# arkworks-rs/accumulation

Hardware: AMD Instinct MI355X
Metric: MSM throughput (point-scalar pairs/sec) at 2^20 Pallas (higher is better)
Workload: dtype u32; 1 GPU; 2^20-pair pallas MSM per GPU (north_star size; scalars uniform in [0, r), G_i = k_i*G), key resident + precomputed window multiples; pairs_per_gpu=1048576, curve=pallas, precomputed_key=True, parallelism=point-sharded x1, window_bits=20, pipeline=bucket-per-lane (k_prep_local_t + k_accum_bpl; skewed scalars re-run chunked), window_widths=9 x 20 + 4 x 19 bits = 256 (MsmGeom::n_narrow), msms_in_flight=3, full=False

## Files before the change

accumulation_amd/csrc/api_entry_ctx.inc:

```

const char* amsm_strerror(int s) {
  switch (s) {
    case AMSM_OK: return "ok";
    case AMSM_E_INVALID_ARG: return "invalid argument";
    case AMSM_E_OOM: return "out of (device) memory";
    case AMSM_E_HIP: return "HIP runtime error";
    case AMSM_E_UNSUPPORTED: return "unsupported size or configuration";
    case AMSM_E_NO_DEVICE: return "no usable gfx950 device (the host backend is never chosen implicitly: ask for AMSM_DEVICE_HOST)";
    case AMSM_E_SCALAR_RANGE: return "scalar out of range (not a canonical into_repr value)";
    case AMSM_E_RCCL: return "RCCL collective failed";
    case AMSM_E_INVALID_POINT: return "invalid point (non-canonical, off the curve or outside the prime-order subgroup)";
    default: return "unknown error";
  }
}

int amsm_device_count(void) {
  int n = 0;
  if (hipGetDeviceCount(&n) != hipSuccess) {
    (void)hipGetLastError();
    return 0;
  }
  return n;
}

// ... 61 lines not shown
  {
    hipDeviceProp_t prop;
    if (hipGetDeviceProperties(&prop, device_id) == hipSuccess && prop.multiProcessorCount > 0) {
      c->cu_count = prop.multiProcessorCount;
      int per_cu = with_curve(curve, [](auto cv) { return accum_l0_blocks_per_cu<typename decltype(cv)::Fq>(); });
      c->wave_slots = prop.multiProcessorCount * std::max(1, per_cu) * 4;
    }
  }
  c->pool_cap_bytes = pool_cap_from_env(c->pool_cap_bytes);
  c->gate.limit = mem_limit_from_env();
  if (const char* e = getenv("AMSM_BPL")) c->bpl = atoi(e) != 0;
  if (const char* e = getenv("AMSM_BPL_PLAIN")) c->bpl_plain = atoi(e) != 0;
  if (const char* e = getenv("AMSM_TOP_SETS")) {
    const int t = atoi(e);
    c->top_sets = (t == 2 || t == 4 || t == 8) ? t : 0;
  }
  if (const char* e = getenv("AMSM_BPL_PROBE")) c->bpl_probe = atoi(e) != 0;
  if (const char* e = getenv("AMSM_BPS")) c->bps = std::max(0, std::min(2, atoi(e)));
  if (const char* e = getenv("AMSM_BPS_BATCH")) c->bps_batch = std::max(0, std::min((int)msel::BPS_BATCH, atoi(e)));
  if (const char* e = getenv("AMSM_SPLIT_LOG2")) c->split_log2 = std::max(0, std::min(28, atoi(e)));
  if (const char* e = getenv("AMSM_DIRECT_SUM_MAX_LOG2")) c->direct_max_log2 = std::max(0, std::min(16, atoi(e)));
  if (const char* e = getenv("AMSM_TWO_VALUED")) c->two_valued = atoi(e) != 0;
  if (const char* e = getenv("AMSM_SHARE_BUCKETS")) c->share_buckets = atoi(e) != 0;
  if (const char* e = getenv("AMSM_HOST_HALVES")) c->host_halves = atoi(e) != 0;
  if (const char* e = getenv("AMSM_SUBGROUP_LADDER")) c->subgroup_ladder = atoi(e) == 2 ? 2 : 1;
  if (const char* e = getenv("AMSM_VEC_SAMPLE_FORM")) c->vec_sample_form = std::max(0, std::min(2, atoi(e)));
  *out = c;
  return AMSM_OK;
}

// ... 282 lines not shown
```

accumulation_amd/csrc/api_pipeline.inc:

```

#define HIP_TRY(expr)                                                                                  \
  do {                                                                                                 \
    hipError_t _e = (expr);                                                                            \
    if (_e != hipSuccess) {                                                                            \
      fprintf(stderr, "[amsm] HIP error %s (%d) at %s:%d: %s\n", hipGetErrorName(_e), (int)_e, __FILE__, \
              __LINE__, #expr);                                                                        \
      return _e == hipErrorOutOfMemory ? AMSM_E_OOM : AMSM_E_HIP;                                      \
    }                                                                                                  \
  } while (0)

#define TRY(expr)            \
  do {                       \
    int _s = (expr);         \
    if (_s != AMSM_OK) return _s; \
  } while (0)

int ensure(DevBuf& b, size_t bytes) {
  if (b.bytes >= bytes && b.p) return AMSM_OK;
  if (b.p) HIP_TRY(gate_free(b.p));
  b.p = nullptr;
  b.bytes = 0;
  size_t want = bytes + bytes / 8 + 256;
  TRY(gate_alloc(b.owner, GATE_DEVICE, want, false, &b.p));
  b.bytes = want;
// ... 473 lines not shown
  u32* d_heavy_count = d_err + 1;
  u32* vals_a = (u32*)sl->vals_a.p;
  u32* vals_b = (u32*)sl->vals_b.p;

  auto prep = [&]() -> int {
    if (!short_prep) HIP_TRY(hipMemsetAsync(sl->misc.p, 0, 64, st));
    stage_mark(ctx, sl, ST_DIGITS, st);
    if (g.bpl) {
      PrepBplBuffers pb;
      pb.d_small = d_err + 16;
      pb.part = vals_a;
      pb.ents_t = vals_b;
      pb.grp = sl->bpl_grp.p;
      pb.order = (u32*)sl->bpl_order.p;
      pb.err = d_err;
      const int rc = g.bpl == 2 ? launch_prep_bps<Fr>(st, (const u32*)d_scalars, scalars_mont, g, g.bps_log2_l, pb)
                                : launch_prep_bpl<Fr>(st, (const u32*)d_scalars, scalars_mont, g, pb);
      if (rc != 0) return AMSM_E_HIP;
      stage_mark(ctx, sl, ST_SORT, st);
      stage_mark(ctx, sl, ST_BOUNDS, st);
      if (g.bpl != 2) ctx->n_bpl++;
      else if (!job.counted) ctx->n_bps++;
      if (g.bpl == 1u && g.top_split) ctx->n_top_sets[(g.top_split + 1u) / 4u]++;
    } else if (short_prep) {
      PrepBuffers pb;
      pb.d_small = d_err + 16;
      pb.part = vals_a;
      pb.vals_sorted = vals_b;
      pb.start = (u32*)sl->start.p;
      pb.items = (u32*)sl->items.p;
// ... 1117 lines not shown
```

accumulation_amd/csrc/api_types.h:

```cpp
#pragma once
struct amsm_ctx;
namespace {

enum Stage { ST_DIGITS = 0, ST_SORT, ST_BOUNDS, ST_ACCUM_L0, ST_ACCUM_L12, ST_REDUCE, ST_COUNT };
const char* kStageNames[ST_COUNT] = {"prep_chain", "prep_sort_rocprim", "prep_bounds_rocprim", "accum_l0", "accum_l1_l2",
                                     "bucket_reduce_fold"};

struct DevBuf {
  void* p = nullptr;
  size_t bytes = 0;
  amsm_ctx* owner = nullptr;
  void release();
};

struct MemGate {
  size_t held = 0, peak = 0;
  size_t limit = 0;
  size_t pinned = 0;
  unsigned long long requests = 0, refused_limit = 0, refused_hook = 0, failed_driver = 0;
  long fail_after = -1;
};

}

// ... 147 lines not shown
struct amsm_ctx {
  int curve = 0;
  int device = 0;
  bool host_only = false;
  hipStream_t stream = nullptr;
  hipStream_t s_prep = nullptr;
  hipStream_t s_tail = nullptr;
  bool own_stream = false;
  int window_override = 0;
  int cu_count = 256;
  unsigned vec_grid_max = 0;
  int wave_slots = 4096;
  bool bpl = true;
  bool bpl_plain = true;
  int top_sets = 0;
  int bps = 2;
  int split_log2 = 21;
  unsigned long long n_bps = 0, n_bps_fallbacks = 0;
  int bps_batch = msel::BPS_BATCH;
  unsigned long long n_bps_units = 0, n_bps_batched = 0, n_bps_unit_reruns = 0;
  unsigned long long n_direct = 0;
  int direct_max_log2 = 15;
  unsigned direct_rr = 0;
  bool host_halves = true;
  bool bpl_probe = true;
  unsigned long long n_top_sets[3] = {0, 0, 0};
  unsigned long long n_bpl = 0, n_bpl_fallbacks = 0;
  bool share_buckets = true;
  DevBuf shared_buckets[2];
  hipEvent_t shared_free[2] = {};
// ... 120 lines not shown
```

accumulation_amd/csrc/kern_fr.hip:

```cpp
#include "launch.h"
#include "vec_kernels.h"
#include "prep_kernels.h"

#include <algorithm>
#include <cmath>
#include <atomic>
#include <cstdlib>
#include <cstring>

namespace amsm {

static inline u32 cdiv_(u32 a, u32 b) { return (a + b - 1) / b; }
void launch_bounds(hipStream_t st, const void* keys_sorted, bool keys16, u32* vals_sorted, MsmGeom g, u32* start,
                   u32* items) {
  if (keys16)
    hipLaunchKernelGGL((k_bounds<uint16_t>), dim3(cdiv_(g.B, 256)), dim3(256), 0, st, (const uint16_t*)keys_sorted,
                       vals_sorted, g, start, items);
  else
    hipLaunchKernelGGL((k_bounds<u32>), dim3(cdiv_(g.B, 256)), dim3(256), 0, st, (const u32*)keys_sorted, vals_sorted,
                       g, start, items);
}

constexpr u32 PREP_MAX_P = 4096;
static PrepGeom prep_geom(const MsmGeom& g) {
// ... 2 lines not shown
  while (((g.B + (1u << pg.SH) - 1u) >> pg.SH) > 512u && pg.SH < 10u) pg.SH++;
  while (((g.B + (1u << pg.SH) - 1u) >> pg.SH) > PREP_MAX_P) pg.SH++;
  pg.P = (g.B + (1u << pg.SH) - 1u) >> pg.SH;
  pg.SPB = g.S <= 16u ? 512u : 256u;
  unsigned long long max_idx = (unsigned long long)g.base_off + g.n - 1ull +
                               (g.precomp ? (unsigned long long)(g.W - 1u) * g.table_stride : 0ull);
  if (g.idx_rel_bits) max_idx = ((unsigned long long)(g.W - 1u) << g.idx_rel_bits) | ((1ull << g.idx_rel_bits) - 1ull);
  pg.IB = 1;
  while ((max_idx >> pg.IB) != 0ull) pg.IB++;
  while (pg.IB + pg.SH > 31u && pg.SH > 0u && ((g.B + (1u << (pg.SH - 1)) - 1u) >> (pg.SH - 1)) <= PREP_MAX_P) pg.SH--;
  pg.P = (g.B + (1u << pg.SH) - 1u) >> pg.SH;
  const u32 budget_words = 37888u, fixed_words = 2u * (1u << pg.SH) + 1024u;
  pg.CAP = budget_words > fixed_words + 4096u ? budget_words - fixed_words : 0u;
  pg.HEAVY = std::max<u32>(4u * (g.E / pg.P + 1u), 1u << 17);
  pg.FIX = 0;
  return pg;
}
static size_t prep_heavy_words(const MsmGeom& g) { return (size_t)g.B + 4096 + 64; }
size_t prep_small_words(const MsmGeom& g) { return 4 * (PREP_MAX_P + 1) + 1 + 3 * prep_heavy_words(g) + PREP_MAX_HEAVY; }
static size_t prep_local_lds(const PrepGeom& pg) { return (2 * (size_t)(1u << pg.SH) + 1024 + pg.CAP) * sizeof(u32); }
constexpr size_t PREP_LDS_LIMIT = 160 * 1024;
static std::atomic<unsigned long long> prep_local_attr_devices{0};
static void prep_local_attr() {
  int dev = 0;
  if (hipGetDevice(&dev) != hipSuccess || dev < 0 || dev >= 64) dev = 63;
  const unsigned long long bit = 1ull << dev;
  if (dev != 63 && (prep_local_attr_devices.load(std::memory_order_acquire) & bit)) return;
  (void)hipFuncSetAttribute((const void*)k_prep_local, hipFuncAttributeMaxDynamicSharedMemorySize, 152 * 1024);
  prep_local_attr_devices.fetch_or(bit, std::memory_order_release);
}
// ... 1 lines not shown
  const size_t cap = (size_t)pg.SPB * g.S;
  return (3 * (size_t)pg.P + cap) * sizeof(u32) + cap * sizeof(uint16_t);
}
bool prep_supported(const MsmGeom& g) {
  if (g.n == 0 || g.S > 32u) return false;
  PrepGeom pg = prep_geom(g);
  return pg.SH <= 12u && pg.IB + pg.SH <= 31u && prep_scatter_lds(g, pg) <= PREP_LDS_LIMIT &&
         prep_local_lds(pg) <= PREP_LDS_LIMIT && (pg.P + 256) * sizeof(u32) <= 64 * 1024;
}

constexpr u32 BPL_LOCAL_FIXED_WORDS = 3u * BPL_NB + 2u * BPL_BINS + 2u * BPL_GROUPS + 2u;
constexpr u32 BPL_LOCAL_BUDGET_WORDS = 40960u;
static_assert(BPL_LOCAL_BUDGET_WORDS - BPL_LOCAL_FIXED_WORDS <= BPL_LOCAL_SLOTS * BPL_NB,
              "k_prep_local_t keeps a partition of CAP entries in BPL_LOCAL_SLOTS registers per lane");
static_assert(BPL_LOCAL_BUDGET_WORDS - BPL_LOCAL_FIXED_WORDS == msel::BPL_STAGE_CAP, "msm_select.h plans for k_prep_local_t's stage");
static PrepGeom prep_bpl_geom(const MsmGeom& g) {
  PrepGeom pg;
  pg.SH = 10;
  pg.P = g.B >> pg.SH;
  pg.SPB = g.S <= 16u ? 512u : 256u;
  unsigned long long max_idx = (unsigned long long)g.base_off + g.n - 1ull +
                               (g.precomp ? (unsigned long long)(g.W - 1u) * g.table_stride : 0ull);
  if (g.idx_rel_bits) max_idx = ((unsigned long long)(g.W - 1u) << g.idx_rel_bits) | ((1ull << g.idx_rel_bits) - 1ull);
  pg.IB = 1;
  while ((max_idx >> pg.IB) != 0ull) pg.IB++;
  pg.CAP = BPL_LOCAL_BUDGET_WORDS - BPL_LOCAL_FIXED_WORDS;
  pg.HEAVY = 0xffffffffu;
  const unsigned long long per = std::max<unsigned long long>(((unsigned long long)g.E + pg.P - 1) / std::max(1u, pg.P), g.part_max);
  pg.FIX = (u32)std::min<unsigned long long>(pg.CAP, (per + per / 4ull + 2048ull + 15ull) & ~15ull);
  return pg;
}
size_t prep_bpl_part_entries(const MsmGeom& g) {
  PrepGeom pg = prep_bpl_geom(g);
  return std::max<size_t>(g.E, pg.FIX ? (size_t)pg.P * pg.FIX : 0);
}
static size_t prep_bpl_local_lds(const PrepGeom& pg) { return (size_t)(BPL_LOCAL_FIXED_WORDS + pg.CAP) * sizeof(u32); }
static size_t prep_bpl_scatter_lds(const MsmGeom& g, const PrepGeom& pg) {
  const size_t cap = (size_t)pg.SPB * g.S;
  return (3 * (size_t)pg.P + 2 * cap) * sizeof(u32) + cap * sizeof(uint16_t);
}
u32 prep_bpl_partitions(const MsmGeom& g) { return g.B >> 10; }
u32 prep_bpl_groups_per_partition() { return BPL_GROUPS; }
u32 prep_bpl_stride(const MsmGeom& g) {
  const u32 P = std::max(1u, prep_bpl_partitions(g));
// ... 6 lines not shown
  PrepGeom pg = prep_bpl_geom(g);
  if (pg.IB > 30u) return false;
  if (!msel::bpl_stage_fits(g.E, pg.P, g.part_max, pg.CAP)) return false;
  return prep_bpl_scatter_lds(g, pg) <= PREP_LDS_LIMIT && prep_bpl_local_lds(pg) <= PREP_LDS_LIMIT &&
         (unsigned long long)pg.P * prep_bpl_stride(g) < (1ull << 31);
}
static std::atomic<unsigned long long> prep_bpl_attr_devices{0};
template <class KS>
static void prep_bpl_attr(KS scatter_kernel) {
  int dev = 0;
  if (hipGetDevice(&dev) != hipSuccess || dev < 0 || dev >= 64) dev = 63;
  const unsigned long long bit = 1ull << dev;
  (void)hipFuncSetAttribute((const void*)scatter_kernel, hipFuncAttributeMaxDynamicSharedMemorySize, (int)PREP_LDS_LIMIT);
  if (dev != 63 && (prep_bpl_attr_devices.load(std::memory_order_acquire) & bit)) return;
  static_assert((BPL_LOCAL_BUDGET_WORDS) * sizeof(u32) <= PREP_LDS_LIMIT, "k_prep_local_t's LDS must fit a workgroup");
  (void)hipFuncSetAttribute((const void*)k_prep_local_t, hipFuncAttributeMaxDynamicSharedMemorySize, (int)PREP_LDS_LIMIT);
  prep_bpl_attr_devices.fetch_or(bit, std::memory_order_release);
}

constexpr u32 bps_local_fixed_words(u32 nbp) { return 4u * nbp + 1024u + BPL_BINS + 2u * BPS_GROUPS + 2u; }
constexpr u32 BPS_LOCAL_BUDGET_WORDS = 37888u;
static PrepGeom prep_bps_geom(const MsmGeom& g, u32 log2_l) {
  PrepGeom pg;
  pg.SH = 10u - log2_l;
  pg.P = g.B >> pg.SH;
  pg.SPB = g.S <= 16u ? 512u : 256u;
  unsigned long long max_idx = (unsigned long long)g.base_off + g.n - 1ull +
                               (g.precomp ? (unsigned long long)(g.W - 1u) * g.table_stride : 0ull);
  if (g.idx_rel_bits) max_idx = ((unsigned long long)(g.W - 1u) << g.idx_rel_bits) | ((1ull << g.idx_rel_bits) - 1ull);
  pg.IB = 1;
  while ((max_idx >> pg.IB) != 0ull) pg.IB++;
  pg.CAP = BPS_LOCAL_BUDGET_WORDS - bps_local_fixed_words(1u << pg.SH);
  pg.HEAVY = 0xffffffffu;
  const unsigned long long per = ((unsigned long long)g.E + pg.P - 1) / std::max(1u, pg.P);
  pg.FIX = (u32)std::min<unsigned long long>(pg.CAP, (per + per / 2ull + 1024ull + 15ull) & ~15ull);
  return pg;
}
size_t prep_bps_part_entries(const MsmGeom& g, u32 log2_l) {
  PrepGeom pg = prep_bps_geom(g, log2_l);
  return std::max<size_t>(g.E, pg.FIX ? (size_t)pg.P * pg.FIX : 0);
}
static size_t prep_bps_local_lds(const PrepGeom& pg) {
  return (size_t)(bps_local_fixed_words(1u << pg.SH) + pg.CAP) * sizeof(u32);
}
u32 prep_bps_partitions(const MsmGeom& g, u32 log2_l) { return g.B >> (10u - log2_l); }
u32 prep_bps_stride(const MsmGeom& g, u32 log2_l) {
  const u32 P = std::max(1u, prep_bps_partitions(g, log2_l));
  const unsigned long long per = ((unsigned long long)g.E + P - 1) / P;
  return (u32)((per + per / 2ull + 4096ull + 1023ull) & ~1023ull);
}
// ... 174 lines not shown
    if (hipMemsetAsync(b.small, 0, (size_t)nv * b.small_stride * sizeof(u32), st) != hipSuccess) return -1;          \
    prep_bps_attr();                                                                                                 \
    const size_t lds_scatter = prep_scatter_lds(g, pg);                                                              \
    if (lds_scatter > 64 * 1024)                                                                                     \
      (void)hipFuncSetAttribute((const void*)k_prep_scatter_batch<FR, 16, 1>, hipFuncAttributeMaxDynamicSharedMemorySize, \
                                (int)PREP_LDS_LIMIT);                                                                \
    hipLaunchKernelGGL((k_prep_scatter_batch<FR, 16, 1>), dim3(cdiv_(g.n, pg.SPB), nv), dim3(512), lds_scatter, st, sc, mont, g,   \
                       pg, part_start0, part_cursor0, b.small_stride, b.part, b.part_stride, b.small);               \
    hipLaunchKernelGGL(k_prep_local_s_batch, dim3(pg.P, nv), dim3(1024), prep_bps_local_lds(pg), st, part_cursor0,   \
                       b.small_stride, b.part, b.part_stride, g, pg, stride, log2_l, b.ents_t, b.ents_stride,        \
                       (BplGroup*)b.grp, b.grp_stride, b.order, b.order_stride, b.small);                            \
    return 0;                                                                                                        \
  }                                                                                                                  \
  template <>                                                                                                        \
  int launch_prep_bpl<FR>(hipStream_t st, const u32* scalars, int mont, MsmGeom g, const PrepBplBuffers& b) {        \
    PrepGeom pg = prep_bpl_geom(g);                                                                                  \
    u32* part_total = b.d_small;                                                                                     \
    u32* part_start = b.d_small + (PREP_MAX_P + 1);                                                                  \
    u32* part_cursor = b.d_small + 2 * (PREP_MAX_P + 1);                                                             \
    PrepHeavy hv;                                                                                                    \
    hv.n = b.d_small + 4 * (PREP_MAX_P + 1);                                                                         \
    hv.cnt = hv.n + 1;                                                                                               \
    hv.ids = hv.cnt + 64;                                  \
    hv.cur = hv.end = hv.ids;                                                                                        \
    {                  \
      size_t zero_bytes = (16 + 4 * (PREP_MAX_P + 1) + 1) * sizeof(u32);                                             \
      zero_bytes = (zero_bytes + 255) & ~(size_t)255;                                                                \
      if (b.err != b.d_small - 16) return -1;                                                                        \
      if (hipMemsetAsync(b.err, 0, zero_bytes, st) != hipSuccess) return -1;                                         \
    }                                                                                                                \
    if (g.S <= 16u) prep_bpl_attr(k_prep_scatter<FR, 16, 1, true>);                                                  \
    else prep_bpl_attr(k_prep_scatter<FR, 32, 1, true>);                                                             \
    if (!pg.FIX) {                                                                                                   \
      PrepGeom ph = pg;                                                                                              \
      ph.SPB = 1024;                                                                                                 \
      hipLaunchKernelGGL((k_prep_hist<FR>), dim3(cdiv_(g.n, 1024)), dim3(1024), pg.P * sizeof(u32), st, scalars,      \
                         mont, g, ph, part_total, b.err);                                                            \
      hipLaunchKernelGGL(k_prep_scan, dim3(1), dim3(1024), 0, st, part_total, part_start, pg.P, pg.HEAVY, hv);       \
    }                                                                                                                \
    if (g.S <= 16u)                                                                                                  \
      hipLaunchKernelGGL((k_prep_scatter<FR, 16, 1, true>), dim3(cdiv_(g.n, pg.SPB)), dim3(512),                     \
                         prep_bpl_scatter_lds(g, pg), st, scalars, mont, g, pg, part_start, part_cursor, b.part, b.err); \
    else                                             \
      hipLaunchKernelGGL((k_prep_scatter<FR, 32, 1, true>), dim3(cdiv_(g.n, pg.SPB)), dim3(256),                     \
                         prep_bpl_scatter_lds(g, pg), st, scalars, mont, g, pg, part_start, part_cursor, b.part, b.err); \
    hipLaunchKernelGGL(k_prep_local_t, dim3(pg.P), dim3(1024), prep_bpl_local_lds(pg), st,                           \
                       pg.FIX ? part_cursor : part_start, (const u64*)b.part, g, pg, prep_bpl_stride(g), b.ents_t,   \
                       (BplGroup*)b.grp, b.order, b.err);                                                            \
    return 0;                                                                                                        \
  }                                                                                                                  \
  template <>                                                                                                        \
  void launch_digits<FR>(hipStream_t st, const u32* scalars, int mont, MsmGeom g, void* keys, bool keys16, u32* vals, \
                         u32* err) {                                                                                 \
    if (keys16)                                                                                                      \
      hipLaunchKernelGGL((k_digits<FR, uint16_t>), dim3(cdiv_(g.n, 256)), dim3(256), 0, st, scalars, mont, g,         \
                         (uint16_t*)keys, vals, err);                                                                \
    else                                                                                                             \
      hipLaunchKernelGGL((k_digits<FR, u32>), dim3(cdiv_(g.n, 256)), dim3(256), 0, st, scalars, mont, g, (u32*)keys,  \
                         vals, err);                                                                                 \
  }                                                                                                                  \
  template <>                                                                                                        \
  void launch_skew_probe<FR>(hipStream_t st, const u32* scalars, int mont, u32 n, DigitWalk walk, u32* d_flag,       \
                             const u32* d_tv_words) {                                                               \
// ... 125 lines not shown
```

accumulation_amd/csrc/launch.h:

```cpp
#pragma once
#include <hip/hip_runtime.h>

#include <algorithm>

#include "blind.h"
#include "msm_select.h"
#include "msm_types.h"

namespace amsm {

template <class Fq>
void launch_accum_l0(hipStream_t st, const u32* table, const u32* vals_sorted, const u32* start,
                     const u32* item_off, MsmGeom g, u32* partials);
template <class Fq>
void launch_accum_bpl(hipStream_t st, const u32* table, const u32* ents_t, const void* grp, const u32* order, u32 n_groups,
                      u32 groups_per_part, const u32* flags, u32* buckets, u32 wg_per_cu = 0, bool accumulate = false);
template <class Fq>
int accum_l0_blocks_per_cu();
template <class Fq>
void launch_accum_l1(hipStream_t st, u32 lanes_per_bucket, const u32* partials, const u32* items, const u32* item_off, MsmGeom g,
                     u32* buckets, u32* heavy_count, u32* heavy_list);
template <class Fq>
void launch_accum_l2(hipStream_t st, const u32* partials, const u32* items, const u32* item_off,
                     const u32* heavy_count, const u32* heavy_list, u32* scratch, u32* buckets);
// ... 63 lines not shown
  u32* part;
  u32* vals_sorted;
  u32* start;
  u32* items;
  u32* item_off;
  u32* err;
};
bool prep_supported(const MsmGeom& g);
struct PrepBplBuffers {
  u32* d_small;
  u32* part;
  u32* ents_t;
  void* grp;
  u32* order;
  u32* err;
};
bool prep_bpl_supported(const MsmGeom& g);
u32 prep_bpl_stride(const MsmGeom& g);
u32 prep_bpl_partitions(const MsmGeom& g);
size_t prep_bpl_part_entries(const MsmGeom& g);
size_t prep_bps_part_entries(const MsmGeom& g, u32 log2_l);
u32 prep_bpl_groups_per_partition();
template <class Fr>
int launch_prep_bpl(hipStream_t st, const u32* scalars, int mont, MsmGeom g, const PrepBplBuffers& b);
int prep_bps_choose(const MsmGeom& g);
u32 prep_bps_partitions(const MsmGeom& g, u32 log2_l);
u32 prep_bps_stride(const MsmGeom& g, u32 log2_l);
template <class Fr>
int launch_prep_bps(hipStream_t st, const u32* scalars, int mont, MsmGeom g, u32 log2_l, const PrepBplBuffers& b);
template <class Fq>
// ... 81 lines not shown
```

accumulation_amd/csrc/msm_select.h:

```cpp
#pragma once
#include <math.h>
#include <stddef.h>

#include <initializer_list>

namespace amsm {
namespace msel {

enum Pipeline { DIRECT_SUM = 0, BUCKET_SPLIT = 1, BUCKET_PER_LANE = 2, CHUNKED = 3 };
inline const char* pipeline_name(int p) {
  return p == DIRECT_SUM ? "direct_sum" : (p == BUCKET_SPLIT ? "bucket_split" : (p == BUCKET_PER_LANE ? "bucket_per_lane" : "chunked"));
}

inline int ilog2_ceil(size_t n) {
  int l = 0;
  while (((size_t)1 << l) < n) l++;
  return l;
}
constexpr size_t P2(int k) { return (size_t)1 << k; }

constexpr int BPL_WINDOW = 20;
constexpr int DIRECT_MAX_LOG2 = 15;
struct KeyWindowRow {
  int lg_lo, lg_hi;
// ... 211 lines not shown
  const unsigned long long per_top = ((unsigned long long)n * 1024ull + reach - 1) / reach;
  const unsigned long long top = (2ull * per_top + T - 1) / T;
  const unsigned long long pm = per_win > top ? per_win : top;
  return groups > 1u ? (pm + 1ull) / 2ull : pm;
}
inline unsigned plain_top_sets(size_t n, unsigned nb, unsigned long long reach, unsigned W, unsigned groups, unsigned cap = BPL_STAGE_CAP,
                               unsigned max_sets = 8) {
  if (n == 0 || nb < 1024u || reach == 0 || W == 0) return 0;
  for (unsigned T = 2; T <= max_sets && T <= 8u; T *= 2u) {
    const unsigned long long P = ((unsigned long long)groups * (W + T) * nb) >> 10;
    if (bpl_stage_fits((unsigned long long)n * W, P, plain_part_max(n, nb, reach, T, groups), cap)) return T;
  }
  return 0;
}
inline unsigned plain_top_sets_cap(int top_sets) { return top_sets == 2 ? 2u : 8u; }

enum class Place {
  LONE,
  BATCH_LAST,
  BATCH_INNER,
};
inline Place place_of(size_t i, size_t count) { return count == 1 ? Place::LONE : (i + 1 == count ? Place::BATCH_LAST : Place::BATCH_INNER); }
enum TailForm {
  RED2 = 0,
  FUSED_QUAD = 1,
  ONE_LANE = 2
};
inline const char* tail_form_name(int f) { return f == RED2 ? "red2" : (f == FUSED_QUAD ? "fused_quad" : "one_lane"); }
constexpr int TAIL_QUAD_HIDDEN_LOG2 = 17;
constexpr unsigned RED2_COLS = 1024, RED2_MIN_NB = 1u << 18;
// ... 65 lines not shown
```

accumulation_amd/csrc/prep_kernels.h:

```cpp
#pragma once
#include "fp.h"
#include "msm_select.h"
#include "msm_types.h"
#include "vec_kernels.h"

namespace amsm {

struct PrepGeom {
  u32 SH;
  u32 P;
  u32 SPB;
  u32 IB;
  u32 CAP;
  u32 HEAVY;
  u32 FIX;
};

constexpr u32 PREP_HEAVY_SLICES = 64, PREP_HEAVY_GRID = 1024, PREP_MAX_HEAVY = 4096;
struct PrepHeavy {
  u32* n;
  u32* ids;
  u32* cnt;
  u32* cur;
  u32* end;
};

constexpr u32 PREP_ENTRY_LAST = 0x40000000u;

AMSM_DEV u32 lds_count(u32* ctr, u32 idx) {
  const u64 active = __ballot(1);
// ... 91 lines not shown
    u32 v = in[k];
    out[k] = run;
    run += v;
  }
  if (with_total && t == T - 1) out[n] = lds[T - 1];
}

__global__ void __launch_bounds__(1024)
    k_prep_scan(const u32* __restrict__ part_total, u32* __restrict__ part_start, u32 P, u32 heavy_min, PrepHeavy hv) {
  __shared__ u32 lds[1024];
  block_exclusive_scan(part_total, part_start, P, true, lds);
  for (u32 p = threadIdx.x; p < P; p += blockDim.x)
    if (part_total[p] > heavy_min) hv.ids[atomicAdd(hv.n, 1u)] = p;
}

template <class Fr, int MAXW, int SPT, bool WIDE>
AMSM_DEV void prep_scatter_body(const u32* scalars, int mont, MsmGeom g, PrepGeom pg, const u32* part_start, u32* part_cursor, u32* part,
                                u32* err) {
  extern __shared__ u32 prep_lds[];
  const u32 cap = pg.SPB * g.S;
  u32* cnt = prep_lds;
  u32* loff = prep_lds + pg.P;
  u32* gbase = prep_lds + 2 * pg.P;
  u32* staged = prep_lds + 3 * pg.P;
  uint16_t* staged_p = reinterpret_cast<uint16_t*>(staged + (WIDE ? 2u : 1u) * cap);
  const u32 t = threadIdx.x, T = blockDim.x;
  for (u32 p = t; p < pg.P; p += T) cnt[p] = 0;
  __syncthreads();
  u32 rk[SPT][MAXW / 2];
  Fe<Fr> sreg[SPT];
// ... 2 lines not shown
#pragma unroll
    for (int k = 0; k < MAXW / 2; k++) rk[r][k] = 0;
    u32 i = blockIdx.x * pg.SPB + r * T + t;
    if (i < g.n) {
      sreg[r] = fe_load<Fr>(scalars + (size_t)i * 8);
      if (g.skip_ones) fe_drop_stored_one<Fr>(sreg[r], mont);
      if (mont) sreg[r] = fe_from_mont<Fr>(sreg[r]);
      const u32 bad = scalar_entries_unrolled_reg<Fr, MAXW>(sreg[r], g, i, [&](int w, u32 key, u32) {
        u32 rank = atomicAdd(&cnt[key >> pg.SH], 1u);
        rk[r][w >> 1] |= rank << ((w & 1) * 16);
      });
      if (pg.FIX && bad && err) atomicOr(err, 1u);
    }
  }
  __syncthreads();
  constexpr u32 RSV_MAX = 4;
  u32 rsv[RSV_MAX], rsv_base[RSV_MAX];
  u32 per = (pg.P + T - 1) / T;
  u32 lo = min(t * per, pg.P), hi = min(lo + per, pg.P);
  {
    u32* sl = reinterpret_cast<u32*>(staged);
    u32 sum = 0;
    for (u32 p = lo; p < hi; p++) sum += cnt[p];
    sl[t] = sum;
    __syncthreads();
    for (u32 d = 1; d < T; d <<= 1) {
      u32 v = t >= d ? sl[t - d] : 0u;
      __syncthreads();
      sl[t] += v;
      __syncthreads();
    }
    u32 run = sl[t] - sum;
#pragma unroll
    for (u32 q = 0; q < RSV_MAX; q++) {
      u32 p = lo + q;
      rsv[q] = 0;
      rsv_base[q] = 0;
      if (p < hi) {
        u32 v = cnt[p];
        loff[p] = run;
        if (v) {
          rsv_base[q] = pg.FIX ? p * pg.FIX : part_start[p];
          rsv[q] = atomicAdd(&part_cursor[p], v);
        }
        run += v;
      }
    }
    for (u32 p = lo + RSV_MAX; p < hi; p++) {
      u32 v = cnt[p];
      loff[p] = run;
      gbase[p] = v ? (pg.FIX ? p * pg.FIX : part_start[p]) + atomicAdd(&part_cursor[p], v) : 0u;
      run += v;
    }
  }
  __syncthreads();
  const u32 low = (1u << pg.SH) - 1u;
#pragma unroll
  for (int r = 0; r < SPT; r++) {
    u32 i = blockIdx.x * pg.SPB + r * T + t;
    if (i < g.n)
      scalar_entries_unrolled_reg<Fr, MAXW>(sreg[r], g, i, [&](int w, u32 key, u32 val) {
        u32 p = key >> pg.SH;
        u32 rank = (rk[r][w >> 1] >> ((w & 1) * 16)) & 0xffffu;
        u32 slot = loff[p] + rank;
        if (WIDE) reinterpret_cast<u64*>(staged)[slot] = ((u64)(key & low) << 32) | val;
        else staged[slot] = (val & 0x80000000u) | ((key & low) << pg.IB) | (val & 0x7fffffffu);
        staged_p[slot] = (uint16_t)p;
      });
  }
#pragma unroll
  for (u32 q = 0; q < RSV_MAX; q++)
    if (lo + q < hi) gbase[lo + q] = rsv_base[q] + rsv[q];
  __syncthreads();
  u32 total = loff[pg.P - 1] + cnt[pg.P - 1];
  for (u32 j = t; j < total; j += T) {
    u32 p = staged_p[j];
    const u32 dst = gbase[p] + (j - loff[p]);
    if (pg.FIX && dst - p * pg.FIX >= pg.FIX) continue;
    if (WIDE) reinterpret_cast<u64*>(part)[dst] = reinterpret_cast<const u64*>(staged)[j];
    else part[dst] = staged[j];
  }
}
template <class Fr, int MAXW, int SPT, bool WIDE = false>
__global__ void __launch_bounds__(512)
    k_prep_scatter(const u32* __restrict__ scalars, int mont, MsmGeom g, PrepGeom pg, const u32* __restrict__ part_start,
                   u32* __restrict__ part_cursor, u32* __restrict__ part, u32* __restrict__ err = nullptr) {
  prep_scatter_body<Fr, MAXW, SPT, WIDE>(scalars, mont, g, pg, part_start, part_cursor, part, err);
}
constexpr int PREP_BPS_BATCH = msel::BPS_BATCH;
struct BpsBatchScalars {
  const u32* scalars[PREP_BPS_BATCH];
};
template <class Fr, int MAXW, int SPT>
// ... 236 lines not shown
  u32 m;
};
AMSM_DEV void bpl_slot(u32 s, u32& pos, u32& half) {
  if (s < BPL_SPLIT) {
    pos = s >> 1;
    half = 1u + (s & 1u);
  } else if (s >= BPL_NB) {
    pos = BPL_SPLIT / 2u + ((s - BPL_NB) >> 1);
    half = 1u + (s & 1u);
  } else {
    pos = s;
    half = 0u;
  }
}

AMSM_DEV u32 block_scan_inclusive(u32 v, u32* wt) {
  const u32 lane = __lane_id(), w = threadIdx.x >> 6;
#pragma unroll
  for (u32 d = 1; d < 64u; d <<= 1) {
    const u32 o = __shfl_up(v, d);
    if (lane >= d) v += o;
  }
  if (lane == 63u) wt[w] = v;
  __syncthreads();
  u32 before = 0;
#pragma unroll
  for (u32 i = 0; i < 15u; i++) before += i < w ? wt[i] : 0u;
  return v + before;
}

constexpr u32 BPL_LOCAL_SLOTS = 37, BPL_SLOT_BLOCK = 8;
template <class F>
AMSM_DEV void bpl_slot_blocks(u32 n, F&& f) {
#pragma unroll
  for (u32 b = 0; b < BPL_LOCAL_SLOTS; b += BPL_SLOT_BLOCK)
    if (b * BPL_NB < n) f(b);
}

__global__ void __launch_bounds__(1024)
    k_prep_local_t(const u32* __restrict__ part_start, const u64* __restrict__ part, MsmGeom g, PrepGeom pg, u32 stride,
                   u32* __restrict__ ents_t, BplGroup* __restrict__ grp, u32* __restrict__ order, u32* __restrict__ err) {
  extern __shared__ u32 prep_lds[];
  constexpr u32 NB = BPL_NB, NG = BPL_GROUPS, T = BPL_NB, SLOTS = BPL_LOCAL_SLOTS, BLK = BPL_SLOT_BLOCK;
  u32* cnt = prep_lds;
  u32* cur = cnt + NB;
  u32* wt = cur + NB;
  u32* bins = wt + NB;
  u32* first = bins + BPL_BINS;
  u32* gm = first + BPL_BINS;
  u32* stage = gm + 2u * NG + 1u;
  const u32 p = blockIdx.x, t = threadIdx.x;
  const u32 ps = pg.FIX ? p * pg.FIX : part_start[p];
  const u32 n_p = pg.FIX ? part_start[p] : part_start[p + 1] - ps;
  const u32 pe = ps + (pg.FIX ? min(n_p, pg.FIX) : n_p);
  const u32 low = NB - 1u, idx_mask = (1u << pg.IB) - 1u, b0 = p << pg.SH;
  const bool fits = n_p <= pg.CAP && (!pg.FIX || n_p <= pg.FIX);
  const u32 n = fits ? min(pe - ps, SLOTS * T) : 0u;
  u64 e[SLOTS];
#pragma unroll
  for (u32 i = 0; i < SLOTS; i++) e[i] = 0;
  bpl_slot_blocks(n, [&](u32 b) {
#pragma unroll
    for (u32 i = b; i < b + BLK && i < SLOTS; i++) e[i] = part[ps + min(i * T + t, n - 1u)];
  });
  cnt[t] = 0;
  if (t < BPL_BINS) bins[t] = 0;
  if (t < NG) gm[t] = 0;
  __syncthreads();
  bpl_slot_blocks(n, [&](u32 b) {
#pragma unroll
    for (u32 i = b; i < b + BLK && i < SLOTS; i++)
      if (i * T + t < n) atomicAdd(&cnt[(u32)(e[i] >> 32) & low], 1u);
  });
  __syncthreads();
  const u32 c_t = cnt[t];
  const u32 first_t = block_scan_inclusive(c_t, wt) - c_t;
  cur[t] = first_t;
  const u32 bin = min(c_t, BPL_BINS - 1u);
  const u32 rank = atomicAdd(&bins[bin], 1u);
  __syncthreads();
  bpl_slot_blocks(n, [&](u32 b) {
    u32 pos[BLK];
#pragma unroll
    for (u32 i = b; i < b + BLK && i < SLOTS; i++) {
      pos[i - b] = 0;
      if (i * T + t < n) pos[i - b] = atomicAdd(&cur[(u32)(e[i] >> 32) & low], 1u);
    }
#pragma unroll
    for (u32 i = b; i < b + BLK && i < SLOTS; i++) {
      const u32 lo = (u32)e[i];
      if (i * T + t < n) stage[pos[i - b]] = (lo & 0x80000000u) | entry_abs_index(g, lo & idx_mask);
    }
  });
  const u32 in_class = t < BPL_BINS ? bins[BPL_BINS - 1u - t] : 0u;
  const u32 larger = block_scan_inclusive(in_class, wt + 16) - in_class;
  if (t < BPL_BINS) first[BPL_BINS - 1u - t] = larger;
  __syncthreads();
  const u32 my_pos = first[bin] + rank;
  cnt[my_pos] = c_t;
  cur[my_pos] = first_t;
  {
    const u32 h0 = (c_t + 1u) >> 1;
    if (my_pos < BPL_SPLIT / 2u) atomicMax(&gm[0], h0);
    else if (my_pos < BPL_SPLIT) atomicMax(&gm[NG - 1u], h0);
    else atomicMax(&gm[my_pos / BPL_GROUP], c_t);
  }
// ... 7 lines not shown
  const bool ok = fits && total <= stride;
  if (!ok && t == 0) atomicOr(err + 1, 1u);
  if (t < NG) {
    BplGroup h;
    h.base = p * stride + my_gb;
    h.m = ok ? gm[t] : 0u;
    grp[p * NG + t] = h;
  }
  {
    u32* o = order + (size_t)p * BPL_LANES;
    if (my_pos < BPL_SPLIT / 2u) o[2u * my_pos] = o[2u * my_pos + 1u] = b0 + t;
    else if (my_pos < BPL_SPLIT) o[BPL_NB + 2u * (my_pos - BPL_SPLIT / 2u)] = o[BPL_NB + 2u * (my_pos - BPL_SPLIT / 2u) + 1u] = b0 + t;
    else o[my_pos] = b0 + t;
  }
  if (!ok) return;
  const u32 w = t >> 6, l = t & 63u;
  auto slot_of = [&](u32 q, u32& sz, u32& src) {
    u32 pos, half;
    bpl_slot(q * BPL_GROUP + l, pos, half);
    const u32 c = cnt[pos], h0 = (c + 1u) >> 1;
    sz = half == 0u ? c : (half == 1u ? h0 : c - h0);
    src = cur[pos] + (half == 2u ? h0 : 0u);
  };
  u32* out = ents_t + (size_t)p * stride + l;
  u32 row0 = 0, sz, src, m = gm[0];
  slot_of(0, sz, src);
  for (u32 q = 0; q < NG; q++) {
    u32 sz_n = 0, src_n = 0, m_n = 0;
    if (q + 1u < NG) {
      m_n = gm[q + 1u];
      slot_of(q + 1u, sz_n, src_n);
// ... 125 lines not shown
```

Baseline: 1.009 billion pairs/s.

## Shard per-partition scatter cursors across blocks to cut global atomic contention

The scatter kernel now splits each fixed-size partition into several sub-regions, each with its own cursor, chosen by block index, so scattering blocks contend on separate global atomic counters. The local transpose kernel gains a sharded variant that rebuilds a per-slot validity mask from the shard counts, because entries are no longer contiguous. The shard count is picked from a statistical margin check on expected fill, and the scatter block scan is replaced with a wave-shuffle scan. The costs are gaps inside partitions, extra validity bookkeeping, and a higher overflow risk for unevenly distributed digits.

```diff
diff --git a/accumulation_amd/csrc/api_entry_ctx.inc b/accumulation_amd/csrc/api_entry_ctx.inc
--- a/accumulation_amd/csrc/api_entry_ctx.inc
+++ b/accumulation_amd/csrc/api_entry_ctx.inc
@@ -99,6 +99,10 @@
   if (const char* e = getenv("AMSM_TOP_SETS")) {
     const int t = atoi(e);
     c->top_sets = (t == 2 || t == 4 || t == 8) ? t : 0;
+  }
+  if (const char* e = getenv("AMSM_PREP_SHARDS")) {
+    const int s = atoi(e);
+    c->prep_shards = (s == 1 || s == 2 || s == 4 || s == 8 || s == 16) ? s : 0;
   }
   if (const char* e = getenv("AMSM_BPL_PROBE")) c->bpl_probe = atoi(e) != 0;
   if (const char* e = getenv("AMSM_BPS")) c->bps = std::max(0, std::min(2, atoi(e)));
diff --git a/accumulation_amd/csrc/api_pipeline.inc b/accumulation_amd/csrc/api_pipeline.inc
--- a/accumulation_amd/csrc/api_pipeline.inc
+++ b/accumulation_amd/csrc/api_pipeline.inc
@@ -511,6 +511,7 @@
       pb.grp = sl->bpl_grp.p;
       pb.order = (u32*)sl->bpl_order.p;
       pb.err = d_err;
+      pb.shards = ctx->prep_shards ? ctx->prep_shards : (one ? 0 : 1);
       const int rc = g.bpl == 2 ? launch_prep_bps<Fr>(st, (const u32*)d_scalars, scalars_mont, g, g.bps_log2_l, pb)
                                 : launch_prep_bpl<Fr>(st, (const u32*)d_scalars, scalars_mont, g, pb);
       if (rc != 0) return AMSM_E_HIP;
diff --git a/accumulation_amd/csrc/api_types.h b/accumulation_amd/csrc/api_types.h
--- a/accumulation_amd/csrc/api_types.h
+++ b/accumulation_amd/csrc/api_types.h
@@ -185,6 +185,7 @@
   bool bpl = true;
   bool bpl_plain = true;
   int top_sets = 0;
+  int prep_shards = 0;
   int bps = 2;
   int split_log2 = 21;
   unsigned long long n_bps = 0, n_bps_fallbacks = 0;
diff --git a/accumulation_amd/csrc/kern_fr.hip b/accumulation_amd/csrc/kern_fr.hip
--- a/accumulation_amd/csrc/kern_fr.hip
+++ b/accumulation_amd/csrc/kern_fr.hip
@@ -40,6 +40,8 @@
   pg.CAP = budget_words > fixed_words + 4096u ? budget_words - fixed_words : 0u;
   pg.HEAVY = std::max<u32>(4u * (g.E / pg.P + 1u), 1u << 17);
   pg.FIX = 0;
+  pg.SHARDS = 1;
+  pg.SUB = 0;
   return pg;
 }
 static size_t prep_heavy_words(const MsmGeom& g) { return (size_t)g.B + 4096 + 64; }
@@ -71,7 +73,8 @@
 static_assert(BPL_LOCAL_BUDGET_WORDS - BPL_LOCAL_FIXED_WORDS <= BPL_LOCAL_SLOTS * BPL_NB,
               "k_prep_local_t keeps a partition of CAP entries in BPL_LOCAL_SLOTS registers per lane");
 static_assert(BPL_LOCAL_BUDGET_WORDS - BPL_LOCAL_FIXED_WORDS == msel::BPL_STAGE_CAP, "msm_select.h plans for k_prep_local_t's stage");
-static PrepGeom prep_bpl_geom(const MsmGeom& g) {
+static_assert(msel::PREP_CURSOR_WORDS == PREP_MAX_P + 1, "msm_select.h keeps the shards' cursors inside the cursor region of d_small");
+static PrepGeom prep_bpl_geom(const MsmGeom& g, int shards = 0) {
   PrepGeom pg;
   pg.SH = 10;
   pg.P = g.B >> pg.SH;
@@ -83,8 +86,11 @@
   while ((max_idx >> pg.IB) != 0ull) pg.IB++;
   pg.CAP = BPL_LOCAL_BUDGET_WORDS - BPL_LOCAL_FIXED_WORDS;
   pg.HEAVY = 0xffffffffu;
-  const unsigned long long per = std::max<unsigned long long>(((unsigned long long)g.E + pg.P - 1) / std::max(1u, pg.P), g.part_max);
-  pg.FIX = (u32)std::min<unsigned long long>(pg.CAP, (per + per / 4ull + 2048ull + 15ull) & ~15ull);
+  pg.FIX = msel::prep_bpl_fix(g.E, pg.P, g.part_max, pg.CAP);
+  const u32 spb_log2 = pg.SPB == 512u ? 9u : 8u;
+  const bool lopsided = g.groups > 1u && g.group_shift >= spb_log2 && g.group_shift < spb_log2 + 4u;
+  pg.SHARDS = lopsided ? 1u : msel::prep_shards(g.E, pg.P, g.part_max, pg.FIX, shards);
+  pg.SUB = msel::prep_shard_sub(pg.FIX, pg.SHARDS);
   return pg;
 }
 size_t prep_bpl_part_entries(const MsmGeom& g) {
@@ -121,7 +127,8 @@
   (void)hipFuncSetAttribute((const void*)scatter_kernel, hipFuncAttributeMaxDynamicSharedMemorySize, (int)PREP_LDS_LIMIT);
   if (dev != 63 && (prep_bpl_attr_devices.load(std::memory_order_acquire) & bit)) return;
   static_assert((BPL_LOCAL_BUDGET_WORDS) * sizeof(u32) <= PREP_LDS_LIMIT, "k_prep_local_t's LDS must fit a workgroup");
-  (void)hipFuncSetAttribute((const void*)k_prep_local_t, hipFuncAttributeMaxDynamicSharedMemorySize, (int)PREP_LDS_LIMIT);
+  (void)hipFuncSetAttribute((const void*)k_prep_local_t<false>, hipFuncAttributeMaxDynamicSharedMemorySize, (int)PREP_LDS_LIMIT);
+  (void)hipFuncSetAttribute((const void*)k_prep_local_t<true>, hipFuncAttributeMaxDynamicSharedMemorySize, (int)PREP_LDS_LIMIT);
   prep_bpl_attr_devices.fetch_or(bit, std::memory_order_release);
 }
 
@@ -141,6 +148,8 @@
   pg.HEAVY = 0xffffffffu;
   const unsigned long long per = ((unsigned long long)g.E + pg.P - 1) / std::max(1u, pg.P);
   pg.FIX = (u32)std::min<unsigned long long>(pg.CAP, (per + per / 2ull + 1024ull + 15ull) & ~15ull);
+  pg.SHARDS = 1;
+  pg.SUB = pg.FIX;
   return pg;
 }
 size_t prep_bps_part_entries(const MsmGeom& g, u32 log2_l) {
@@ -345,16 +354,17 @@
   }                                                                                                                  \
   template <>                                                                                                        \
   int launch_prep_bpl<FR>(hipStream_t st, const u32* scalars, int mont, MsmGeom g, const PrepBplBuffers& b) {        \
-    PrepGeom pg = prep_bpl_geom(g);                                                                                  \
+    PrepGeom pg = prep_bpl_geom(g, b.shards);                                                                        \
     u32* part_total = b.d_small;                                                                                     \
     u32* part_start = b.d_small + (PREP_MAX_P + 1);                                                                  \
-    u32* part_cursor = b.d_small + 2 * (PREP_MAX_P + 1);                                                             \
+    u32* part_cursor = b.d_small + 2 * (PREP_MAX_P + 1);   \
     PrepHeavy hv;                                                                                                    \
     hv.n = b.d_small + 4 * (PREP_MAX_P + 1);                                                                         \
     hv.cnt = hv.n + 1;                                                                                               \
     hv.ids = hv.cnt + 64;                                  \
     hv.cur = hv.end = hv.ids;                                                                                        \
-    {                  \
+    if ((size_t)pg.SHARDS * pg.P > PREP_MAX_P + 1 || (size_t)pg.SHARDS * pg.SUB > pg.FIX) return -1;                 \
+    {   \
       size_t zero_bytes = (16 + 4 * (PREP_MAX_P + 1) + 1) * sizeof(u32);                                             \
       zero_bytes = (zero_bytes + 255) & ~(size_t)255;                                                                \
       if (b.err != b.d_small - 16) return -1;                                                                        \
@@ -375,9 +385,13 @@
     else                                             \
       hipLaunchKernelGGL((k_prep_scatter<FR, 32, 1, true>), dim3(cdiv_(g.n, pg.SPB)), dim3(256),                     \
                          prep_bpl_scatter_lds(g, pg), st, scalars, mont, g, pg, part_start, part_cursor, b.part, b.err); \
-    hipLaunchKernelGGL(k_prep_local_t, dim3(pg.P), dim3(1024), prep_bpl_local_lds(pg), st,                           \
-                       pg.FIX ? part_cursor : part_start, (const u64*)b.part, g, pg, prep_bpl_stride(g), b.ents_t,   \
-                       (BplGroup*)b.grp, b.order, b.err);                                                            \
+    if (pg.SHARDS > 1u)                                                                                              \
+      hipLaunchKernelGGL(k_prep_local_t<true>, dim3(pg.P), dim3(1024), prep_bpl_local_lds(pg), st, part_cursor,      \
+                         (const u64*)b.part, g, pg, prep_bpl_stride(g), b.ents_t, (BplGroup*)b.grp, b.order, b.err); \
+    else                                                                                                             \
+      hipLaunchKernelGGL(k_prep_local_t<false>, dim3(pg.P), dim3(1024), prep_bpl_local_lds(pg), st,                  \
+                         pg.FIX ? part_cursor : part_start, (const u64*)b.part, g, pg, prep_bpl_stride(g), b.ents_t, \
+                         (BplGroup*)b.grp, b.order, b.err);                                                          \
     return 0;                                                                                                        \
   }                                                                                                                  \
   template <>                                                                                                        \
diff --git a/accumulation_amd/csrc/launch.h b/accumulation_amd/csrc/launch.h
--- a/accumulation_amd/csrc/launch.h
+++ b/accumulation_amd/csrc/launch.h
@@ -101,6 +101,7 @@
   void* grp;
   u32* order;
   u32* err;
+  int shards = 0;
 };
 bool prep_bpl_supported(const MsmGeom& g);
 u32 prep_bpl_stride(const MsmGeom& g);
diff --git a/accumulation_amd/csrc/msm_select.h b/accumulation_amd/csrc/msm_select.h
--- a/accumulation_amd/csrc/msm_select.h
+++ b/accumulation_amd/csrc/msm_select.h
@@ -249,6 +249,36 @@
   return 0;
 }
 inline unsigned plain_top_sets_cap(int top_sets) { return top_sets == 2 ? 2u : 8u; }
+
+inline unsigned prep_bpl_fix(unsigned long long E, unsigned long long P, unsigned long long part_max, unsigned cap) {
+  const unsigned long long avg = (E + P - 1) / (P ? P : 1ull), per = avg > part_max ? avg : part_max;
+  const unsigned long long want = (per + per / 4ull + 2048ull + 15ull) & ~15ull;
+  return (unsigned)(want < cap ? want : cap);
+}
+constexpr unsigned PREP_CURSOR_WORDS = 4096 + 1;
+constexpr unsigned PREP_SHARDS_MAX = 8;
+inline unsigned prep_shard_sub(unsigned fix, unsigned S) { return S <= 1u ? fix : (fix / S) & ~63u; }
+inline bool prep_shards_hard(unsigned S, unsigned long long P, unsigned fix, unsigned cursor_words) {
+  if (S == 1u) return true;
+  if (S != 2u && S != 4u && S != 8u && S != 16u) return false;
+  const unsigned sub = prep_shard_sub(fix, S);
+  return sub != 0u && (unsigned long long)S * sub <= fix && (unsigned long long)S * P <= cursor_words;
+}
+inline bool prep_shards_margin(unsigned S, unsigned long long E, unsigned long long P, unsigned long long part_max, unsigned fix) {
+  if (S == 1u) return true;
+  const unsigned long long avg = (E + P - 1) / (P ? P : 1ull), per = avg > part_max ? avg : part_max;
+  const double fill = (double)per / S;
+  return (double)prep_shard_sub(fix, S) >= fill + 6.0 * sqrt(fill);
+}
+inline unsigned prep_shards(unsigned long long E, unsigned long long P, unsigned long long part_max, unsigned fix, int forced = 0,
+                            unsigned cursor_words = PREP_CURSOR_WORDS, unsigned s_max = PREP_SHARDS_MAX) {
+  const bool f = forced == 1 || forced == 2 || forced == 4 || forced == 8 || forced == 16;
+  for (unsigned S = f ? (unsigned)forced : 16u; S > 1u; S /= 2u) {
+    if (!f && S > s_max) continue;
+    if (prep_shards_hard(S, P, fix, cursor_words) && (f || prep_shards_margin(S, E, P, part_max, fix))) return S;
+  }
+  return 1u;
+}
 
 enum class Place {
   LONE,
diff --git a/accumulation_amd/csrc/prep_kernels.h b/accumulation_amd/csrc/prep_kernels.h
--- a/accumulation_amd/csrc/prep_kernels.h
+++ b/accumulation_amd/csrc/prep_kernels.h
@@ -14,6 +14,7 @@
   u32 CAP;
   u32 HEAVY;
   u32 FIX;
+  u32 SHARDS, SUB;
 };
 
 constexpr u32 PREP_HEAVY_SLICES = 64, PREP_HEAVY_GRID = 1024, PREP_MAX_HEAVY = 4096;
@@ -135,6 +136,21 @@
     if (part_total[p] > heavy_min) hv.ids[atomicAdd(hv.n, 1u)] = p;
 }
 
+AMSM_DEV u32 block_scan_inclusive(u32 v, u32* wt) {
+  const u32 lane = __lane_id(), w = threadIdx.x >> 6;
+#pragma unroll
+  for (u32 d = 1; d < 64u; d <<= 1) {
+    const u32 o = __shfl_up(v, d);
+    if (lane >= d) v += o;
+  }
+  if (lane == 63u) wt[w] = v;
+  __syncthreads();
+  u32 before = 0;
+#pragma unroll
+  for (u32 i = 0; i < 15u; i++) before += i < w ? wt[i] : 0u;
+  return v + before;
+}
+
 template <class Fr, int MAXW, int SPT, bool WIDE>
 AMSM_DEV void prep_scatter_body(const u32* scalars, int mont, MsmGeom g, PrepGeom pg, const u32* part_start, u32* part_cursor, u32* part,
                                 u32* err) {
@@ -167,6 +183,10 @@
     }
   }
   __syncthreads();
+  const u32 shard = (WIDE && pg.SHARDS > 1u) ? (blockIdx.x & (pg.SHARDS - 1u)) : 0u;
+  const u32 shard_off = shard * pg.SUB;
+  const u32 room = (WIDE && pg.SHARDS > 1u) ? pg.SUB : pg.FIX;
+  if (WIDE) part_cursor += shard * pg.P;
   constexpr u32 RSV_MAX = 4;
   u32 rsv[RSV_MAX], rsv_base[RSV_MAX];
   u32 per = (pg.P + T - 1) / T;
@@ -175,15 +195,7 @@
     u32* sl = reinterpret_cast<u32*>(staged);
     u32 sum = 0;
     for (u32 p = lo; p < hi; p++) sum += cnt[p];
-    sl[t] = sum;
-    __syncthreads();
-    for (u32 d = 1; d < T; d <<= 1) {
-      u32 v = t >= d ? sl[t - d] : 0u;
-      __syncthreads();
-      sl[t] += v;
-      __syncthreads();
-    }
-    u32 run = sl[t] - sum;
+    u32 run = block_scan_inclusive(sum, sl) - sum;
 #pragma unroll
     for (u32 q = 0; q < RSV_MAX; q++) {
       u32 p = lo + q;
@@ -193,7 +205,7 @@
         u32 v = cnt[p];
         loff[p] = run;
         if (v) {
-          rsv_base[q] = pg.FIX ? p * pg.FIX : part_start[p];
+          rsv_base[q] = pg.FIX ? p * pg.FIX + shard_off : part_start[p];
           rsv[q] = atomicAdd(&part_cursor[p], v);
         }
         run += v;
@@ -202,7 +214,7 @@
     for (u32 p = lo + RSV_MAX; p < hi; p++) {
       u32 v = cnt[p];
       loff[p] = run;
-      gbase[p] = v ? (pg.FIX ? p * pg.FIX : part_start[p]) + atomicAdd(&part_cursor[p], v) : 0u;
+      gbase[p] = v ? (pg.FIX ? p * pg.FIX + shard_off : part_start[p]) + atomicAdd(&part_cursor[p], v) : 0u;
       run += v;
     }
   }
@@ -229,7 +241,7 @@
   for (u32 j = t; j < total; j += T) {
     u32 p = staged_p[j];
     const u32 dst = gbase[p] + (j - loff[p]);
-    if (pg.FIX && dst - p * pg.FIX >= pg.FIX) continue;
+    if (pg.FIX && dst - (p * pg.FIX + shard_off) >= room) continue;
     if (WIDE) reinterpret_cast<u64*>(part)[dst] = reinterpret_cast<const u64*>(staged)[j];
     else part[dst] = staged[j];
   }
@@ -496,22 +508,8 @@
   }
 }
 
-AMSM_DEV u32 block_scan_inclusive(u32 v, u32* wt) {
-  const u32 lane = __lane_id(), w = threadIdx.x >> 6;
-#pragma unroll
-  for (u32 d = 1; d < 64u; d <<= 1) {
-    const u32 o = __shfl_up(v, d);
-    if (lane >= d) v += o;
-  }
-  if (lane == 63u) wt[w] = v;
-  __syncthreads();
-  u32 before = 0;
-#pragma unroll
-  for (u32 i = 0; i < 15u; i++) before += i < w ? wt[i] : 0u;
-  return v + before;
-}
-
 constexpr u32 BPL_LOCAL_SLOTS = 37, BPL_SLOT_BLOCK = 8;
+constexpr u32 PREP_SHARDS_LIMIT = 16;
 template <class F>
 AMSM_DEV void bpl_slot_blocks(u32 n, F&& f) {
 #pragma unroll
@@ -519,6 +517,7 @@
     if (b * BPL_NB < n) f(b);
 }
 
+template <bool SHARDED>
 __global__ void __launch_bounds__(1024)
     k_prep_local_t(const u32* __restrict__ part_start, const u64* __restrict__ part, MsmGeom g, PrepGeom pg, u32 stride,
                    u32* __restrict__ ents_t, BplGroup* __restrict__ grp, u32* __restrict__ order, u32* __restrict__ err) {
@@ -531,28 +530,74 @@
   u32* first = bins + BPL_BINS;
   u32* gm = first + BPL_BINS;
   u32* stage = gm + 2u * NG + 1u;
-  const u32 p = blockIdx.x, t = threadIdx.x;
+  u32* vcnt = wt + 32u;
+  static_assert(32u + SLOTS * 16u <= NB, "the validity table lies in the words set aside behind the wave totals");
+  const u32 p = blockIdx.x, t = threadIdx.x, w = t >> 6, l = t & 63u;
   const u32 ps = pg.FIX ? p * pg.FIX : part_start[p];
-  const u32 n_p = pg.FIX ? part_start[p] : part_start[p + 1] - ps;
-  const u32 pe = ps + (pg.FIX ? min(n_p, pg.FIX) : n_p);
   const u32 low = NB - 1u, idx_mask = (1u << pg.IB) - 1u, b0 = p << pg.SH;
-  const bool fits = n_p <= pg.CAP && (!pg.FIX || n_p <= pg.FIX);
-  const u32 n = fits ? min(pe - ps, SLOTS * T) : 0u;
   u64 e[SLOTS];
-#pragma unroll
-  for (u32 i = 0; i < SLOTS; i++) e[i] = 0;
+  u64 valid = 0;
+  u32 n;
+  bool fits;
+  if constexpr (!SHARDED) {
+    const u32 n_p = pg.FIX ? part_start[p] : part_start[p + 1] - ps;
+    const u32 pe = ps + (pg.FIX ? min(n_p, pg.FIX) : n_p);
+    fits = n_p <= pg.CAP && (!pg.FIX || n_p <= pg.FIX);
+    n = fits ? min(pe - ps, SLOTS * T) : 0u;
+#pragma unroll
+    for (u32 i = 0; i < SLOTS; i++) e[i] = 0;
+    bpl_slot_blocks(n, [&](u32 b) {
+#pragma unroll
+      for (u32 i = b; i < b + BLK && i < SLOTS; i++) e[i] = part[ps + min(i * T + t, n - 1u)];
+    });
+    cnt[t] = 0;
+    if (t < BPL_BINS) bins[t] = 0;
+    if (t < NG) gm[t] = 0;
+    __syncthreads();
+  } else {
+    u32 n_p = 0, n_end = 0;
+    bool over = false;
+#pragma unroll
+    for (u32 s = 0; s < PREP_SHARDS_LIMIT; s++) {
+      const u32 v = part_start[min(s, pg.SHARDS - 1u) * pg.P + p];
+      const u32 c = s < pg.SHARDS ? v : 0u;
+      n_p += c;
+      over = over || c > pg.SUB;
+      if (c) n_end = s * pg.SUB + c;
+    }
+    fits = n_p <= pg.CAP && !over;
+    n = fits ? min(n_end, SLOTS * T) : 0u;
+    if (t < SLOTS * 16u) {
+      const u32 pos0 = t * 64u;
+      u32 v = 0;
+      if (pos0 < n) {
+        const u32 s = pos0 / pg.SUB, r0 = pos0 - s * pg.SUB;
+        const u32 c = part_start[s * pg.P + p];
+        v = c > r0 ? min(c - r0, 64u) : 0u;
+      }
+      vcnt[t] = v;
+    }
+    cnt[t] = 0;
+    if (t < BPL_BINS) bins[t] = 0;
+    if (t < NG) gm[t] = 0;
+    __syncthreads();
+    bpl_slot_blocks(n, [&](u32 b) {
+#pragma unroll
+      for (u32 i = b; i < b + BLK && i < SLOTS; i++)
+        if (l < vcnt[i * 16u + w]) valid |= 1ull << i;
+    });
+#pragma unroll
+    for (u32 i = 0; i < SLOTS; i++) e[i] = 0;
+    bpl_slot_blocks(n, [&](u32 b) {
+#pragma unroll
+      for (u32 i = b; i < b + BLK && i < SLOTS; i++) e[i] = part[ps + (((valid >> i) & 1ull) ? i * T + t : n - 1u)];
+    });
+  }
+  auto holds = [&](u32 i) { return SHARDED ? ((valid >> i) & 1ull) != 0ull : i * T + t < n; };
   bpl_slot_blocks(n, [&](u32 b) {
 #pragma unroll
-    for (u32 i = b; i < b + BLK && i < SLOTS; i++) e[i] = part[ps + min(i * T + t, n - 1u)];
-  });
-  cnt[t] = 0;
-  if (t < BPL_BINS) bins[t] = 0;
-  if (t < NG) gm[t] = 0;
-  __syncthreads();
-  bpl_slot_blocks(n, [&](u32 b) {
-#pragma unroll
     for (u32 i = b; i < b + BLK && i < SLOTS; i++)
-      if (i * T + t < n) atomicAdd(&cnt[(u32)(e[i] >> 32) & low], 1u);
+      if (holds(i)) atomicAdd(&cnt[(u32)(e[i] >> 32) & low], 1u);
   });
   __syncthreads();
   const u32 c_t = cnt[t];
@@ -566,12 +611,12 @@
 #pragma unroll
     for (u32 i = b; i < b + BLK && i < SLOTS; i++) {
       pos[i - b] = 0;
-      if (i * T + t < n) pos[i - b] = atomicAdd(&cur[(u32)(e[i] >> 32) & low], 1u);
+      if (holds(i)) pos[i - b] = atomicAdd(&cur[(u32)(e[i] >> 32) & low], 1u);
     }
 #pragma unroll
     for (u32 i = b; i < b + BLK && i < SLOTS; i++) {
       const u32 lo = (u32)e[i];
-      if (i * T + t < n) stage[pos[i - b]] = (lo & 0x80000000u) | entry_abs_index(g, lo & idx_mask);
+      if (holds(i)) stage[pos[i - b]] = (lo & 0x80000000u) | entry_abs_index(g, lo & idx_mask);
     }
   });
   const u32 in_class = t < BPL_BINS ? bins[BPL_BINS - 1u - t] : 0u;
@@ -609,7 +654,6 @@
     else o[my_pos] = b0 + t;
   }
   if (!ok) return;
-  const u32 w = t >> 6, l = t & 63u;
   auto slot_of = [&](u32 q, u32& sz, u32& src) {
     u32 pos, half;
     bpl_slot(q * BPL_GROUP + l, pos, half);
```

Result: slower. 989.1 million pairs/s (-2.0%).
